# penn-pal-lab/robot_aware_control

Measured on AMD Instinct MI355X. Metric: SVG train frames/sec + CEM candidate-rollouts/sec, 64x64, higher is better.
Workload: dtype fp32 (conv operands as two fp16 parts = 22 significant bits, fp32 accumulate; see fp32_exact)

## Files before the change

### robot_aware_control_amd/csrc/rac_split16.hip

```cpp
#include <math.h>
#include <stdlib.h>

#include <type_traits>

#include "rac_common.h"

namespace rac {

typedef _Float16 f16x8 __attribute__((ext_vector_type(8)));
typedef _Float16 f16x4 __attribute__((ext_vector_type(4)));
typedef unsigned int u32x4 __attribute__((ext_vector_type(4)));
typedef unsigned int u32x2 __attribute__((ext_vector_type(2)));
typedef __amdgpu_buffer_rsrc_t rsrc_t;

constexpr unsigned OOB = 0xFFFFFFF0u;
constexpr int SBN = 128, SBK = 32;

__device__ __forceinline__ const void* uniform_ptr(const void* p) {
  unsigned long long v = reinterpret_cast<unsigned long long>(p);
  unsigned lo = __builtin_amdgcn_readfirstlane((unsigned)v);
  unsigned hi = __builtin_amdgcn_readfirstlane((unsigned)(v >> 32));
  return reinterpret_cast<const void*>(((unsigned long long)hi << 32) | lo);
}
__device__ __forceinline__ rsrc_t make_rsrc(const void* p, unsigned bytes) {
// ... 1535 lines not shown
        __builtin_amdgcn_sched_barrier(0);
        f16x8 fb[NB][2];
#pragma unroll
        for (int j2 = 0; j2 < NT; ++j2)
#pragma unroll
          for (int nb = 0; nb < 2; ++nb)
#pragma unroll
            for (int part = 0; part < 2; ++part)
              fb[j2 * 2 + nb][part] = __builtin_bit_cast(f16x8, bs[tap % 3][(j2 * 2 + part) * 2 + nb]);
        if (!(RAC_EXP_PERSIST & 8) || tap == 0) {
#pragma unroll
          for (int t = HB; t < MB; ++t) read_frag(t, tap, cur * abuf);
        }
        __builtin_amdgcn_sched_barrier(0);
#pragma unroll
        for (int t = 0; t < HB; ++t)
#pragma unroll
          for (int nb = 0; nb < NB; ++nb) acc[t][nb] = mma3(fa[t], fb[nb], acc[t][nb]);
        __builtin_amdgcn_sched_barrier(0);
        if (tap == 8 && more) {
          store_a(cur ^ 1, pow2f(cur_t.ka));
          __syncthreads();
          cur ^= 1;
        }
        if ((tap < 8 || more) && (!(RAC_EXP_PERSIST & 8) || tap == 8)) {
#pragma unroll
          for (int t = 0; t < HB; ++t) read_frag(t, (tap + 1) % 9, cur * abuf);
        }
        __builtin_amdgcn_sched_barrier(0);
#pragma unroll
        for (int t = HB; t < MB; ++t)
#pragma unroll
          for (int nb = 0; nb < NB; ++nb) acc[t][nb] = mma3(fa[t], fb[nb], acc[t][nb]);
      }
    }
    const int img = p.per_image ? cur_t.m0 / p.HW : 0;
    if (RAC_EXP_PERSIST & 2) {
      unsigned mx = 0;
#pragma unroll
      for (int i = 0; i < MB; ++i)
#pragma unroll
        for (int j = 0; j < NB; ++j)
#pragma unroll
          for (int r = 0; r < 4; ++r) mx = max(mx, absbits(acc[i][j][r]));
      if (p.out_amax) amax_commit(mx, p.out_amax + img);
    } else {
      conv16_epilogue(p, acc, cur_t.m0, wm * MB, nmb, n0 + wn * NT * 32, 0, pow2f(-cur_t.ka), pow2f(-kw), pre, nullptr,
                      p.out_amax ? p.out_amax + img : nullptr);
    }
    if (!has_next) break;
    cur ^= 1;
    cur_t = nxt_t;
    bx = next_bx;
  }
}

__global__ __launch_bounds__(256) void absmax_kernel(const float4* x0, long n0v, const float4* x1, long n1v,
                                                     unsigned* amax) {
  __shared__ unsigned sh[4];
  unsigned m = 0;
  const long stride = (long)gridDim.x * blockDim.x;
  for (long i = (long)blockIdx.x * blockDim.x + threadIdx.x; i < n0v + n1v; i += stride) {
    const float4 v = i < n0v ? x0[i] : x1[i - n0v];
    const unsigned a = __builtin_bit_cast(unsigned, v.x) & 0x7FFFFFFFu, b = __builtin_bit_cast(unsigned, v.y) & 0x7FFFFFFFu,
                   c = __builtin_bit_cast(unsigned, v.z) & 0x7FFFFFFFu, d = __builtin_bit_cast(unsigned, v.w) & 0x7FFFFFFFu;
    m = max(m, max(max(a, b), max(c, d)));
  }
#pragma unroll
  for (int o = 32; o > 0; o >>= 1) m = max(m, (unsigned)__shfl_xor((int)m, o));
  if ((threadIdx.x & 63) == 0) sh[threadIdx.x >> 6] = m;
  __syncthreads();
  if (threadIdx.x == 0) {
    m = max(max(sh[0], sh[1]), max(sh[2], sh[3]));
    if (m > __hip_atomic_load(amax, __ATOMIC_RELAXED, __HIP_MEMORY_SCOPE_AGENT)) atomicMax(amax, m);
  }
}

__device__ __forceinline__ void weight_frag16_block(const float* w, const unsigned* w_amax, unsigned short* out, int Cout,
                                                    int Cin, int taps, int transposed, long ps, long block) {
  const int R = transposed ? Cin : Cout, Kc = transposed ? Cout : Cin;
  const int cch = Kc >> 5;
  const long cell = block * 2 + (threadIdx.x >> 7);
  if (cell >= (long)(R >> 5) * cch * taps) return;
  const float s = pow2f(scale_exp(*w_amax));
  const int tap = (int)(cell % taps);
  const int cc = (int)((cell / taps) % cch);
  const int nt = (int)(cell / ((long)taps * cch));
  const int nb = (threadIdx.x >> 6) & 1, lane = threadIdx.x & 63;
  const int r = nt * 32 + nb * 16 + (lane & 15);
  const int k0 = cc * 32 + 8 * (lane >> 4);
  u32x4 lo, hi;
  if (!transposed) {
    const u32x4* src = reinterpret_cast<const u32x4*>(w + ((long)r * taps + tap) * Cin + k0);
    lo = src[0], hi = src[1];
  } else {
    unsigned v[8];
#pragma unroll
    for (int j = 0; j < 8; ++j)
      v[j] = __builtin_bit_cast(unsigned, w[((long)(k0 + j) * taps + (taps - 1 - tap)) * Cin + r]);
    lo = u32x4{v[0], v[1], v[2], v[3]}, hi = u32x4{v[4], v[5], v[6], v[7]};
  }
  u32x4 q[2];
  split8h(lo, hi, s, q);
  const long o = (cell * 2 + nb) * 512 + lane * 8;
  *reinterpret_cast<u32x4*>(out + o) = q[0];
  *reinterpret_cast<u32x4*>(out + ps + o) = q[1];
}

__global__ void weight_frag16_kernel(const float* w, const unsigned* w_amax, unsigned short* out, int Cout, int Cin,
                                     int taps, int transposed, long ps) {
  weight_frag16_block(w, w_amax, out, Cout, Cin, taps, transposed, ps, blockIdx.x);
}

template <typename Job>
__device__ __forceinline__ int job_of_block(const Job* jobs, int n_jobs, long block) {
  int lo = 0, hi = n_jobs - 1;
  while (lo < hi) {
    const int mid = (lo + hi + 1) >> 1;
    if (jobs[mid].block_begin <= block) lo = mid; else hi = mid - 1;
  }
  return lo;
}

__global__ void weight_frag16_multi_kernel(const rac_frag_job* jobs, int n_jobs) {
  const int j = job_of_block(jobs, n_jobs, blockIdx.x);
  const rac_frag_job q = jobs[j];
  weight_frag16_block(q.w, q.w_amax, q.parts, q.Cout, q.Cin, q.ksize * q.ksize, q.transposed, q.part_stride,
                      blockIdx.x - q.block_begin);
}

__global__ __launch_bounds__(256) void absmax_multi_kernel(const rac_absmax_job* jobs, int n_jobs) {
  __shared__ unsigned sh[4];
  const int j = job_of_block(jobs, n_jobs, blockIdx.x);
  const rac_absmax_job q = jobs[j];
  const long nb = (j + 1 < n_jobs ? jobs[j + 1].block_begin : (long)gridDim.x) - q.block_begin;
  const float4* x = reinterpret_cast<const float4*>(q.x);
  const long nv = q.n >> 2;
  unsigned m = 0;
  for (long i = (blockIdx.x - q.block_begin) * 256 + threadIdx.x; i < nv; i += nb * 256) {
    const float4 v = x[i];
    m = max(m, max(max(absbits(v.x), absbits(v.y)), max(absbits(v.z), absbits(v.w))));
  }
#pragma unroll
  for (int o = 32; o > 0; o >>= 1) m = max(m, (unsigned)__shfl_xor((int)m, o));
  if ((threadIdx.x & 63) == 0) sh[threadIdx.x >> 6] = m;
  __syncthreads();
  if (threadIdx.x == 0) {
    m = max(max(sh[0], sh[1]), max(sh[2], sh[3]));
    if (m > __hip_atomic_load(q.amax, __ATOMIC_RELAXED, __HIP_MEMORY_SCOPE_AGENT)) atomicMax(q.amax, m);
  }
}


__global__ __launch_bounds__(256) void adam_frag_multi_kernel(const rac_adam_frag_job* jobs, int n_jobs, long total_blocks,
                                                              float b1, float b2, float eps, float step_size,
                                                              float inv_sqrt_bc2) {
  __shared__ float tile[2][32][33];
  __shared__ unsigned mx_sh[4];
  for (long blk = blockIdx.x; blk < total_blocks; blk += gridDim.x) {
  const int j = job_of_block(jobs, n_jobs, (int)blk);
  const rac_adam_frag_job q = jobs[j];
  const int taps = q.ksize * q.ksize, cch = q.Cin >> 5;
  const int half = threadIdx.x >> 7;
  const long cell = (blk - q.block_begin) * 2 + half;
  const bool active = cell < (long)(q.Cout >> 5) * cch * taps;
  const int tap = (int)(cell % taps);
  const int cc = (int)((cell / taps) % cch);
  const int nt = (int)(cell / ((long)taps * cch));
  const int nb = (threadIdx.x >> 6) & 1, lane = threadIdx.x & 63;
  const int rl = nb * 16 + (lane & 15), kl = 8 * (lane >> 4);
  const float s = pow2f(scale_exp(*q.scale_slot));
  unsigned mx = 0;
  if (active) {
    const long off = ((long)(nt * 32 + rl) * taps + tap) * q.Cin + cc * 32 + kl;
    f32x4 P[2], G[2], M[2], V[2];
#pragma unroll
    for (int h = 0; h < 2; ++h) {
      P[h] = *reinterpret_cast<const f32x4*>(q.p + off + 4 * h);
      G[h] = *reinterpret_cast<const f32x4*>(q.g + off + 4 * h);
      M[h] = *reinterpret_cast<const f32x4*>(q.m + off + 4 * h);
      V[h] = *reinterpret_cast<const f32x4*>(q.v + off + 4 * h);
#pragma unroll
      for (int e = 0; e < 4; ++e) {
        float pp = P[h][e], mm = M[h][e], vv = V[h][e];
        adam_update(pp, G[h][e], mm, vv, b1, b2, eps, step_size, inv_sqrt_bc2);
        M[h][e] = mm, V[h][e] = vv, P[h][e] = pp;
        mx = max(mx, absbits(pp));
        tile[half][rl][kl + 4 * h + e] = pp;
      }
      *reinterpret_cast<f32x4*>(q.p + off + 4 * h) = P[h];
      *reinterpret_cast<f32x4*>(q.m + off + 4 * h) = M[h];
      *reinterpret_cast<f32x4*>(q.v + off + 4 * h) = V[h];
    }
    if (q.parts_fwd) {
      u32x4 parts[2];
      split8h(__builtin_bit_cast(u32x4, P[0]), __builtin_bit_cast(u32x4, P[1]), s, parts);
      const long o = (cell * 2 + nb) * 512 + lane * 8;
      *reinterpret_cast<u32x4*>(q.parts_fwd + o) = parts[0];
      *reinterpret_cast<u32x4*>(q.parts_fwd + q.part_stride + o) = parts[1];
    }
  }
  __syncthreads();
  if (active && q.parts_t) {
    float v[8];
#pragma unroll
    for (int e = 0; e < 8; ++e) v[e] = tile[half][kl + e][rl];
    u32x4 parts[2];
    split8h(u32x4{__builtin_bit_cast(unsigned, v[0]), __builtin_bit_cast(unsigned, v[1]), __builtin_bit_cast(unsigned, v[2]),
                  __builtin_bit_cast(unsigned, v[3])},
            u32x4{__builtin_bit_cast(unsigned, v[4]), __builtin_bit_cast(unsigned, v[5]), __builtin_bit_cast(unsigned, v[6]),
                  __builtin_bit_cast(unsigned, v[7])}, s, parts);
    const long cell_t = ((long)cc * (q.Cout >> 5) + nt) * taps + (taps - 1 - tap);
    const long o = (cell_t * 2 + nb) * 512 + lane * 8;
    *reinterpret_cast<u32x4*>(q.parts_t + o) = parts[0];
    *reinterpret_cast<u32x4*>(q.parts_t + q.part_stride + o) = parts[1];
  }
#pragma unroll
  for (int o = 32; o > 0; o >>= 1) mx = max(mx, (unsigned)__shfl_xor((int)mx, o));
  if (lane == 0) mx_sh[threadIdx.x >> 6] = mx;
  __syncthreads();
  if (threadIdx.x == 0) {
    mx = max(max(mx_sh[0], mx_sh[1]), max(mx_sh[2], mx_sh[3]));
    if (mx > __hip_atomic_load(q.amax_out, __ATOMIC_RELAXED, __HIP_MEMORY_SCOPE_AGENT)) atomicMax(q.amax_out, mx);
  }
  }
}

__global__ void amax_bound_kernel(unsigned* exact, unsigned* bound, const int* idx, int n, float margin) {
  const int j = blockIdx.x * blockDim.x + threadIdx.x;
  if (j >= n) return;
  const int i = idx[j];
  bound[i] = __builtin_bit_cast(unsigned, __builtin_bit_cast(float, exact[i]) + margin);
  exact[i] = 0;
}


struct Wgrad16P {
  int Bimg, H, W, Cin, Cout, C0, T;
  int R, G;
  int nsplit, accumulate;
  int nseg;
  int x1_skip;
  int presplit;
  const float* dy[RAC_WGRAD_MAX_STEPS];
  const float* x0[RAC_WGRAD_MAX_STEPS];
  const float* x1[RAC_WGRAD_MAX_STEPS];
  const unsigned* dy_amax[RAC_WGRAD_MAX_STEPS];
  const unsigned* x0_amax[RAC_WGRAD_MAX_STEPS];
  const unsigned* x1_amax[RAC_WGRAD_MAX_STEPS];
  float* dw;
  float* slabs;
  long slab_stride;
};

typedef __fp16 h16x4 __attribute__((__vector_size__(4 * sizeof(__fp16))));
#define RAC_LDS_PTR(T, base, off) reinterpret_cast<__attribute__((address_space(3))) T*>( \
    (__attribute__((address_space(3))) unsigned char*)(base) + (off))

__device__ __forceinline__ int wg_swz(int r) { return (r & 3) | (((r >> 3) & 1) << 2); }

__device__ __forceinline__ f16x8 tr_frag(const unsigned char* lds, int addr) {
  typedef __fp16 h16x8 __attribute__((__vector_size__(8 * sizeof(__fp16))));
  const h16x4 lo = __builtin_amdgcn_ds_read_tr16_b64_v4f16(RAC_LDS_PTR(h16x4, lds, addr));
  const h16x4 hi = __builtin_amdgcn_ds_read_tr16_b64_v4f16(RAC_LDS_PTR(h16x4, lds, addr + 1024));
  return __builtin_bit_cast(f16x8, (h16x8)__builtin_shufflevector(lo, hi, 0, 1, 2, 3, 4, 5, 6, 7));
}

template <int N>
struct StepPhase {
  static constexpr int v = N;
};
constexpr unsigned OOBV = 0xFFFFFF00u;

__device__ __forceinline__ u32x4 load16s(rsrc_t r, unsigned voff, unsigned soff) {
  return __builtin_bit_cast(u32x4, __builtin_amdgcn_raw_buffer_load_b128(r, (int)voff, (int)soff, 0));
}

template <int KS, int WMW, bool PRE>
__global__ __launch_bounds__(256, 2) void wgrad16_kernel(Wgrad16P p) {
  constexpr int PAD = KS / 2, NR = 2 * PAD + 2;
  constexpr int AHEAD = (KS == 5 && WMW == 2) ? 1 : 2;
  constexpr int DYB = 16384, XSLOT = 8192, X_BASE = 2 * DYB;
  constexpr unsigned EB = PRE ? 2u : 4u;
  static_assert(NR % 2 == 0, "the dy buffer index is a function of the ring phase");
  extern __shared__ __attribute__((aligned(16))) unsigned char lds_raw[];
  const int tid = threadIdx.x;
  const int lane = tid & 63;
  const int wid = __builtin_amdgcn_readfirstlane(tid >> 6);
  constexpr int WN = 4 / WMW, NU = 4 / WN;
  const int wm = wid / WN, wn = wid % WN;
  const int co0 = blockIdx.x * (64 * WMW), ci0 = blockIdx.y * 64;
  const int ky = blockIdx.z % KS, split = blockIdx.z / KS;
  const bool first = ci0 < p.C0;
  const int Cs = first ? p.C0 : p.Cin - p.C0;
  const int cl0 = first ? ci0 : ci0 - p.C0;

  float sd = 1.f, sx = 1.f;
  int kd, kxs;
  {
    unsigned amd = 0, amx = 0;
    for (int t = 0; t < p.T; ++t) {
      amd = max(amd, *p.dy_amax[t]);
      amx = max(amx, *p.x0_amax[t]);
      if (p.x1_amax[t]) amx = max(amx, *p.x1_amax[t]);
    }
    kd = scale_exp(amd), kxs = scale_exp(amx);
    sd = pow2f(kd), sx = pow2f(kxs);
  }

  const int g_skip = first ? 0 : p.x1_skip * p.G;
  const int NG = p.T * p.G;
  const int gpb = (NG - g_skip + p.nsplit - 1) / p.nsplit;
  const int g_begin = g_skip + split * gpb;
  const int g_end = min(NG, g_begin + gpb);
  const int S = max(0, g_end - g_begin) * p.W;

  const int skk = tid >> 3, ssub = tid & 7;
  const int ssw = wg_swz(skk);
  const bool dy_role = WMW == 2 || wid < 2;
  const int dkk = WMW == 2 ? skk : (tid >> 2) & 31, dsub = WMW == 2 ? ssub : tid & 3;
  const int dsw = wg_swz(dkk);
  const int dy_lds = dkk * 256 + ((dsub ^ dsw) * 32);
  const unsigned dflip = (unsigned)(WMW == 2 ? ((dsub ^ dsw) >> 2) & 1 : dkk & 1) * 16u;
  const int x_lds = X_BASE + skk * 256 + (((ssub >> 1) ^ ssw) * 32) + (ssub & 1) * 16;
  const bool dy_ch_ok = co0 + dsub * 16 < p.Cout;
  const bool x_ch_ok = cl0 + ssub * 8 < Cs;

  const unsigned dy_col = (unsigned)p.Cout * EB, dy_row = (unsigned)p.W * dy_col, dy_grp = 32u * dy_row;
  const unsigned dy_part = PRE ? (unsigned)((long)p.R * dy_row) : 0u;
  const unsigned dy_lane = ((unsigned)(dkk * p.W) * (unsigned)p.Cout + (unsigned)(co0 + dsub * 16)) * EB;
  const unsigned d_v0 = dy_ch_ok ? dy_lane + (PRE ? dflip : 2u * dflip) : OOBV;
  const unsigned d_v1 = dy_ch_ok ? dy_lane + (PRE ? (dflip ^ 16u) : (32u ^ (2u * dflip))) : OOBV;
  const unsigned x_col = (unsigned)Cs * EB, x_row = (unsigned)p.W * x_col, x_grp = 32u * x_row;
  const unsigned x_part = PRE ? (unsigned)((long)p.R * x_row) : 0u;
  const unsigned x_lane = ((unsigned)(skk * p.W) * (unsigned)Cs + (unsigned)(cl0 + ssub * 8)) * EB;
  const long x_shift = (long)(ky - PAD) * (long)x_row;
  const bool h32 = __builtin_amdgcn_readfirstlane((32 % p.H) == 0 ? 1 : 0) != 0;
  const bool y_ok0 = (unsigned)(skk % p.H + ky - PAD) < (unsigned)p.H;
  const float* const* xsrc = first ? p.x0 : p.x1;

  int dT = g_begin / p.G, dG = g_begin - dT * p.G, dC = 0;
  int xT = dT, xG = dG, xC = 0;
  rsrc_t d_rs = make_rsrc(p.dy[0], 0u), x_rs = d_rs, d_rs1 = d_rs, x_rs1 = d_rs;
  unsigned d_so = 0, x_so = 0;
  unsigned x_v = (x_ch_ok & (y_ok0 | !h32)) ? x_lane : OOBV;
  u32x4 rdS[AHEAD][4], rxS[AHEAD][2];
  auto issue_dy = [&](u32x4 (&rd)[4]) {
    if (dC == 0) {
      const char* base = reinterpret_cast<const char*>(p.dy[dT]) + (long)dG * dy_grp;
      d_rs = make_rsrc(base, (unsigned)(p.R - dG * 32) * dy_row);
      if constexpr (PRE) d_rs1 = make_rsrc(base + dy_part, (unsigned)(p.R - dG * 32) * dy_row);
      d_so = 0;
    }
    if (dy_role) {
      if constexpr (PRE) {
        rd[0] = load16s(d_rs, d_v0, d_so);
        rd[1] = load16s(d_rs, d_v1, d_so);
        rd[2] = load16s(d_rs1, d_v0, d_so);
        rd[3] = load16s(d_rs1, d_v1, d_so);
      } else {
        rd[0] = load16s(d_rs, d_v0, d_so);
        rd[1] = load16s(d_rs, d_v0 + 16u, d_so);
        rd[2] = load16s(d_rs, d_v1, d_so);
        rd[3] = load16s(d_rs, d_v1 + 16u, d_so);
      }
    }
    d_so += dy_col;
    if (++dC == p.W) {
      dC = 0;
      if (++dG == p.G) dG = 0, ++dT;
    }
  };
  auto issue_x = [&](u32x4 (&rx)[2]) {
    if (xC == 0) {
      const char* base = reinterpret_cast<const char*>(xsrc[xT]) + ((long)xG * x_grp + x_shift);
      x_rs = make_rsrc(base, (unsigned)(p.R - xG * 32) * x_row);
      if constexpr (PRE) x_rs1 = make_rsrc(base + x_part, (unsigned)(p.R - xG * 32) * x_row);
// ... 960 lines not shown
```

### robot_aware_control_amd/ops.py

```python
from __future__ import annotations

import contextlib
import ctypes as C
import functools
import os
import weakref
from typing import Optional, Tuple

import torch

from . import _lib
from ._lib import (AbsmaxJob, AdamFragJob, AdamRange, ConvArgs, FragJob, GradSrc, OptimRange, WgradArgs, call, ptr,
                   stream_ptr)

FWD, DGRAD, WGRAD = 0, 1, 2
ACT_NONE, ACT_LEAKY, ACT_SIGMOID = 0, 1, 2
LOSS_KINDS = {"mse": 0, "l1": 1, "dontcare_mse": 2, "dontcare_l1": 3}
BN_EPS, BN_MOMENTUM = 1e-5, 0.1


def _require_cuda(t: torch.Tensor):
    if not t.is_cuda:
        raise _lib.RacError("robot_aware_control_amd ops run on the GPU only (no CPU fallback); got a CPU tensor")

# ... 243 lines not shown
    M = dy.numel() // dy.shape[-1]
    if _WINDOW is not None and M <= _COLSUM_STEPS_MAX_ROWS:
        _WINDOW.biases.setdefault(id(bias), (bias, []))[1].append(dy)
        return
    call("rac_colsum_acc", ptr(dy), ptr(grad_buffer(bias)), ptr(_colsum_parts(dy.device, M, dy.shape[-1])), M,
         dy.shape[-1], stream_ptr())


def _colsum_parts(device, M: int, Cc: int):
    return torch.empty(int(_lib.load().rac_colsum_blocks(M, Cc)) * Cc, device=device, dtype=torch.float32)


_COLSUM_STEPS_MAX_ROWS = 16384


SPLIT_GEMM = os.environ.get("RAC_SPLIT_GEMM", "1") == "1"
SPLIT_GEMM_TRAIN = SPLIT_GEMM
HEAD_DIRECT = os.environ.get("RAC_HEAD_DIRECT", "1") == "1"
FIRST_MFMA = os.environ.get("RAC_FIRST_MFMA", "1") == "1"
HEAD_DGRAD = os.environ.get("RAC_HEAD_DGRAD", "1") == "1"
HEAD_MFMA = os.environ.get("RAC_HEAD_MFMA", "1") == "1"
SPLIT_MIN_COUT = int(os.environ.get("RAC_SPLIT_MIN_COUT", "64"))
SPLIT_MIN_COUT_TRAIN = int(os.environ.get("RAC_SPLIT_MIN_COUT_TRAIN", "64"))

_AMAX = {"buf": None, "used": 0, "one": None}
_AMAX_SLOTS = 1 << 20


def _amax_take(device, n: int) -> torch.Tensor:
    buf = _AMAX["buf"]
    if buf is None or buf.device != torch.device(device) or _AMAX["used"] + n > _AMAX_SLOTS:
        buf = _AMAX["buf"] = torch.zeros(max(_AMAX_SLOTS, n), device=device, dtype=torch.int32)
        _AMAX["used"] = 0
    k = _AMAX["used"]
    _AMAX["used"] = k + n
    return buf[k:k + n]


def amax_of(x0: torch.Tensor, x1: Optional[torch.Tensor] = None, per_image: bool = False) -> torch.Tensor:
    if per_image:
        assert x1 is None
        slot = _amax_take(x0.device, x0.shape[0])
        call("rac_absmax_rows", ptr(x0), x0.shape[0], x0.numel() // x0.shape[0], ptr(slot), stream_ptr())
        return slot
    slot = _amax_take(x0.device, 1)
    call("rac_absmax", ptr(x0), x0.numel(), ptr(x1), x1.numel() if x1 is not None else 0, ptr(slot), stream_ptr())
    return slot


def amax_slot(device, n: int = 1) -> torch.Tensor:
    return _amax_take(device, n)


def amax_one(device, n: int = 1) -> torch.Tensor:
    one = _AMAX["one"]
    if one is None or one.device != torch.device(device) or one.numel() < n:
        one = _AMAX["one"] = torch.full((max(n, 1024),), 0x3F800000, device=device, dtype=torch.int32)
    view = one[:n]
    view._rac_bound1 = True
    return view


def tag_amax(t: torch.Tensor, slot: torch.Tensor) -> torch.Tensor:
    t._rac_amax = slot
    t._rac_amax_ver = t._version
    return t


def amax_tag(t):
    if t is None or getattr(t, "_rac_amax_ver", None) != t._version:
        return None
    return getattr(t, "_rac_amax", None)


def retag(t, slot):
    if t is not None and slot is not None:
        t._rac_amax = slot
        t._rac_amax_ver = t._version
    return t


def amax_for(t: torch.Tensor, per_image: bool = False) -> torch.Tensor:
    slot = amax_tag(t)
    want = t.shape[0] if per_image else 1
    if slot is not None and getattr(slot, "_rac_bound1", False):
        return amax_one(t.device, want)
    if slot is None or slot.numel() != want:
        slot = amax_of(t, per_image=per_image)
        tag_amax(t, slot)
    return slot


def broadcast_images(t: torch.Tensor, n: int) -> torch.Tensor:
    out = t.expand(n, *t.shape[1:]).contiguous()
    slot = amax_tag(t)
    if slot is not None:
        if getattr(slot, "_rac_bound1", False):
            tag_amax(out, amax_one(t.device, n))
        elif slot.numel() == 1:
            tag_amax(out, slot.expand(n).contiguous())
    return out


_SPLIT_OK = {}


def split_supported(H: int, W: int, k: int, Cin: int, Cout: int, a_split: int = 0) -> bool:
    key = (H, W, k, Cin, Cout, a_split)
    ok = _SPLIT_OK.get(key)
    if ok is None:
        ok = _SPLIT_OK[key] = bool(_lib.load().rac_conv2d_split_supported(H, W, k, Cin, Cout, a_split))
    return ok


class _WeightParts:
    __slots__ = ("ref", "idx", "slot", "device", "parts", "tag", "exact_ok", "__weakref__")


_WP_ENTRIES = {}
_WP_DEV = {}
_WP_NSLOTS = 1024


def _wp_state(device):
    st = _WP_DEV.get(device)
    if st is None:
        st = _WP_DEV[device] = {"slots": torch.zeros(_WP_NSLOTS, device=device, dtype=torch.int32),
                                "exact": torch.zeros(_WP_NSLOTS, device=device, dtype=torch.int32),
                                "free": list(range(_WP_NSLOTS - 1, -1, -1)), "tables": {}, "adam_plan": None,
                                "optim_plan": None}
    return st


def _wp_drop(key, device, idx, _ref):
    ent = _WP_ENTRIES.get(key)
    if ent is not None and ent.idx == idx and ent.device == device:
        del _WP_ENTRIES[key]
        st = _WP_DEV.get(device)
        if st is not None:
            st["free"].append(idx)


def _wp_tag(weight):
    src = getattr(weight, "_rac_sources", None)
    ver = weight._version if src is None else tuple(t._version for t in src)
    return (ver, PARAM_EPOCH, weight.data_ptr())


def _wp_upload(jobs, device):
    raw = bytes(jobs)
    return torch.frombuffer(bytearray(raw), dtype=torch.uint8).to(device)


ADAM_LATE_WGS = int(os.environ.get("RAC_ADAM_LATE_WGS", "512"))
ADAM_WGS = int(os.environ.get("RAC_ADAM_WGS", "0"))


PARAM_GATE = None


def param_wait(t: torch.Tensor = None) -> None:
    gate = PARAM_GATE
    if gate is None:
        return
    if t is None:
        gate.wait_params()
    elif hasattr(gate, "wait_for"):
        gate.wait_for(t)
    elif not gate.ready(t):
        gate.wait_params()


def _wp_tables(st, items, device):
    lib = _lib.load()
    sig = tuple((w.data_ptr(), ent.idx, tuple(sorted((t, q.data_ptr()) for t, q in ent.parts.items())))
                for ent, w in items)
    tables = st["tables"].get(sig)
    if tables is None:
        if len(st["tables"]) > 8:
            st["tables"].clear()
        ajobs = (AbsmaxJob * len(items))()
        nfrag = sum(len(ent.parts) for ent, _ in items)
        fjobs = (FragJob * nfrag)()
        ab = fb = j = 0
        for i, (ent, w) in enumerate(items):
            wm = weight_mem(w.detach())
            co, ci, k, _ = w.shape
            ajobs[i] = AbsmaxJob(x=ptr(wm), n=wm.numel(), amax=ptr(ent.slot), block_begin=ab)
            ab += lib.rac_absmax_blocks(wm.numel())
            for transposed, parts in sorted(ent.parts.items()):
                fjobs[j] = FragJob(w=ptr(wm), w_amax=ptr(ent.slot), parts=ptr(parts), part_stride=wm.numel(), Cout=co,
                                   Cin=ci, ksize=k, transposed=1 if transposed else 0, block_begin=fb)
                fb += lib.rac_weight_frag_blocks(co, ci, k)
                j += 1
        idx = torch.tensor([ent.idx for ent, _ in items], device=device, dtype=torch.long)
        tables = st["tables"][sig] = (_wp_upload(ajobs, device), len(items), ab, _wp_upload(fjobs, device), nfrag, fb, idx)
    return tables


def _wp_refresh(device):
    st = _wp_state(device)
    stale, n_live = [], 0
    gate = PARAM_GATE
    for ent in list(_WP_ENTRIES.values()):
        if ent.device != device:
            continue
        w = ent.ref()
        if w is None:
            continue
        src = getattr(w, "_rac_pad_source", None)
        if gate is not None:
            base = src[0]() if src is not None else w
            if base is not None and not gate.ready(base):
                continue
        if src is not None:
            param = src[0]()
            if param is None:
                continue
            padded_weight(param, src[1])
        n_live += 1
        if ent.tag != _wp_tag(w):
            stale.append((ent, w))
    if not stale:
        return
    sp = stream_ptr()
    if len(stale) <= 2:
        for ent, w in stale:
            ent.slot.zero_()
            wm = weight_mem(w.detach())
            co, ci, k, _ = w.shape
            call("rac_absmax", ptr(wm), wm.numel(), None, 0, ptr(ent.slot), sp)
            for transposed, parts in ent.parts.items():
                call("rac_weight_frag_split", ptr(wm), ptr(ent.slot), ptr(parts), co, ci, k, 1 if transposed else 0,
                     wm.numel(), sp)
            st["exact"][ent.idx:ent.idx + 1].copy_(ent.slot)
            ent.tag, ent.exact_ok = _wp_tag(w), True
        return
    ta, na, ab, tf, nf, fb, idx = _wp_tables(st, stale, device)
    st["slots"].index_fill_(0, idx, 0)
    call("rac_absmax_multi", ptr(ta), na, ab, sp)
    call("rac_weight_frag_split_multi", ptr(tf), nf, fb, sp)
    st["exact"].index_copy_(0, idx, st["slots"].index_select(0, idx))
    for ent, w in stale:
        ent.tag, ent.exact_ok = _wp_tag(w), True


ADAM_FUSED = os.environ.get("RAC_ADAM_FUSED", "1") == "1"
_ADAM_BOUNDS = {}


def adam_step_bound(beta1: float, beta2: float):
    key = (beta1, beta2)
    if key not in _ADAM_BOUNDS:
        r = beta1 * beta1 / beta2
        if not (0.0 <= beta1 < 1.0 and 0.0 < beta2 < 1.0 and r < 1.0):
            _ADAM_BOUNDS[key] = None
        else:
            best, series, b1t, b2t, rk = 0.0, 0.0, 1.0, 1.0, 1.0
            for _ in range(200000):
                series += rk
                rk *= r
                b1t *= beta1
                b2t *= beta2
                best = max(best, (1 - beta1) ** 2 / (1 - b1t) ** 2 * (1 - b2t) / (1 - beta2) * series)
                if rk < 1e-18 and b1t < 1e-18 and b2t < 1e-9:
                    break
            _ADAM_BOUNDS[key] = best ** 0.5
    return _ADAM_BOUNDS[key]


def _wp_covered(flat):
    dev = flat.device
    base, nbytes = flat.data_ptr(), flat.numel() * 4
    covered = []
    for ent in _WP_ENTRIES.values():
        if ent.device != dev:
            continue
        w = ent.ref()
        if w is None or getattr(w, "_rac_pad_source", None) is not None:
            continue
        off = w.data_ptr() - base
        co, ci, k, _ = w.shape
        if not (0 <= off < nbytes and off % 16 == 0 and w.stride() == (k * k * ci, 1, k * ci, ci)):
            continue
        if ent.tag != _wp_tag(w) or not ent.exact_ok:
            return None
        covered.append((off // 4, ent, w))
    covered.sort(key=lambda c: c[0])
    return covered


def fused_adam_step(flat, grad, m, v, lr, beta1, beta2, eps, step, late=None):
    global PARAM_EPOCH
    if not ADAM_FUSED:
        return False
    bound = adam_step_bound(beta1, beta2)
    if bound is None:
        return False
    dev = flat.device
    st = _wp_state(dev)
    base = flat.data_ptr()
    covered = _wp_covered(flat)
    if not covered:
        return False
    late_sets = [] if late is None else (list(late[1]) if isinstance(late[1], (list, tuple)) else [late[1]])

    def late_group(off, w):
# ... 2396 lines not shown
```

Measured before the change: 4133.

## Software-pipeline Adam fragment kernel loads across grid-stride iterations

The Adam fragment kernel's grid-stride loop is restructured so the next block's parameters, gradients and moments are prefetched into registers while the current block is updated. Job lookup is cached and re-seeked only when a block crosses into a new job. The per-block amax reduction and atomic are deferred until the job changes, and the memory access mapping is changed to coalesced row strides. Gradients are loaded and split parts stored with nontemporal hints. The late-launch workgroup count drops from 512 to 256, which gives each workgroup more iterations to pipeline but lowers parallelism and raises register pressure.

Measured after the change: 4166 (median of 4 runs). About the same (+0.8%).

```diff
diff --git a/robot_aware_control_amd/csrc/rac_split16.hip b/robot_aware_control_amd/csrc/rac_split16.hip
--- a/robot_aware_control_amd/csrc/rac_split16.hip
+++ b/robot_aware_control_amd/csrc/rac_split16.hip
@@ -1711,77 +1711,147 @@
 }
 
 
-__global__ __launch_bounds__(256) void adam_frag_multi_kernel(const rac_adam_frag_job* jobs, int n_jobs, long total_blocks,
-                                                              float b1, float b2, float eps, float step_size,
-                                                              float inv_sqrt_bc2) {
+__device__ __forceinline__ void adam_barrier() {
+  __builtin_amdgcn_fence(__ATOMIC_RELEASE, "workgroup");
+  __builtin_amdgcn_s_barrier();
+  __builtin_amdgcn_fence(__ATOMIC_ACQUIRE, "workgroup");
+}
+__device__ __forceinline__ unsigned adam_lane_xor(unsigned v, int o) {
+  return (unsigned)__builtin_amdgcn_ds_bpermute((int)(((threadIdx.x & 63) ^ o) << 2), (int)v);
+}
+template <typename T, typename U>
+__device__ __forceinline__ __attribute__((address_space(1))) T* gmem(U* p) {
+  return (__attribute__((address_space(1))) T*)p;
+}
+
+struct adam_walk {
+  rac_adam_frag_job q;
+  long end;
+  float s;
+  int j;
+};
+struct adam_cell {
+  long cell, off, step;
+  int tap, cc, nt;
+  bool active;
+};
+struct adam_regs {
+  f32x4 P[2], G[2], M[2], V[2];
+};
+
+__device__ __forceinline__ void adam_walk_seek(adam_walk& w, const rac_adam_frag_job* __restrict__ jobs, int n_jobs,
+                                               long total_blocks, long blk) {
+  w.j = job_of_block(jobs, n_jobs, blk);
+  w.q = jobs[w.j];
+  w.end = w.j + 1 < n_jobs ? jobs[w.j + 1].block_begin : total_blocks;
+  w.s = pow2f(scale_exp(*gmem<const unsigned>(w.q.scale_slot)));
+}
+
+__device__ __forceinline__ adam_cell adam_cell_of(const rac_adam_frag_job& q, long blk, int half, int lr, int lc) {
+  adam_cell c;
+  const unsigned taps = q.ksize * q.ksize, cch = q.Cin >> 5;
+  const unsigned cell = (unsigned)(blk - q.block_begin) * 2u + half;
+  c.active = cell < (unsigned long)(q.Cout >> 5) * cch * taps;
+  c.tap = (int)(cell % taps), c.cc = (int)((cell / taps) % cch), c.nt = (int)(cell / (taps * cch));
+  c.cell = cell;
+  c.off = ((long)(c.nt * 32 + lr) * taps + c.tap) * q.Cin + c.cc * 32 + lc;
+  c.step = 16L * taps * q.Cin;
+  return c;
+}
+
+__device__ __forceinline__ void adam_fetch(adam_regs& d, const rac_adam_frag_job& q, const adam_cell& c) {
+  if (!c.active) return;
+#pragma unroll
+  for (int h = 0; h < 2; ++h) {
+    const long o = c.off + h * c.step;
+    d.P[h] = *gmem<const f32x4>(q.p + o);
+    d.G[h] = __builtin_nontemporal_load(gmem<const f32x4>(q.g + o));
+    d.M[h] = *gmem<const f32x4>(q.m + o);
+    d.V[h] = *gmem<const f32x4>(q.v + o);
+  }
+}
+
+__device__ __forceinline__ void adam_parts_out(const float (*tile)[33], bool t, int rl, int kl, float s, unsigned short* out,
+                                               long part_stride, long o) {
+  unsigned v[8];
+#pragma unroll
+  for (int e = 0; e < 8; ++e) v[e] = __builtin_bit_cast(unsigned, t ? tile[kl + e][rl] : tile[rl][kl + e]);
+  u32x4 parts[2];
+  split8h(u32x4{v[0], v[1], v[2], v[3]}, u32x4{v[4], v[5], v[6], v[7]}, s, parts);
+  __builtin_nontemporal_store(parts[0], gmem<u32x4>(out + o));
+  __builtin_nontemporal_store(parts[1], gmem<u32x4>(out + part_stride + o));
+}
+
+__global__ __launch_bounds__(256) void adam_frag_multi_kernel(const rac_adam_frag_job* __restrict__ jobs, int n_jobs,
+                                                              long total_blocks, float b1, float b2, float eps,
+                                                              float step_size, float inv_sqrt_bc2) {
   __shared__ float tile[2][32][33];
   __shared__ unsigned mx_sh[4];
-  for (long blk = blockIdx.x; blk < total_blocks; blk += gridDim.x) {
-  const int j = job_of_block(jobs, n_jobs, (int)blk);
-  const rac_adam_frag_job q = jobs[j];
-  const int taps = q.ksize * q.ksize, cch = q.Cin >> 5;
-  const int half = threadIdx.x >> 7;
-  const long cell = (blk - q.block_begin) * 2 + half;
-  const bool active = cell < (long)(q.Cout >> 5) * cch * taps;
-  const int tap = (int)(cell % taps);
-  const int cc = (int)((cell / taps) % cch);
-  const int nt = (int)(cell / ((long)taps * cch));
-  const int nb = (threadIdx.x >> 6) & 1, lane = threadIdx.x & 63;
+  const int half = threadIdx.x >> 7, nb = (threadIdx.x >> 6) & 1, lane = threadIdx.x & 63;
   const int rl = nb * 16 + (lane & 15), kl = 8 * (lane >> 4);
-  const float s = pow2f(scale_exp(*q.scale_slot));
+  const int lr = (threadIdx.x & 127) >> 3, lc = 4 * (threadIdx.x & 7);
+  long blk = blockIdx.x;
+  if (blk >= total_blocks) return;
+  adam_walk wn;
+  adam_walk_seek(wn, jobs, n_jobs, total_blocks, blk);
+  adam_cell cn = adam_cell_of(wn.q, blk, half, lr, lc);
+  adam_regs dn{};
+  adam_fetch(dn, wn.q, cn);
   unsigned mx = 0;
-  if (active) {
-    const long off = ((long)(nt * 32 + rl) * taps + tap) * q.Cin + cc * 32 + kl;
-    f32x4 P[2], G[2], M[2], V[2];
-#pragma unroll
-    for (int h = 0; h < 2; ++h) {
-      P[h] = *reinterpret_cast<const f32x4*>(q.p + off + 4 * h);
-      G[h] = *reinterpret_cast<const f32x4*>(q.g + off + 4 * h);
-      M[h] = *reinterpret_cast<const f32x4*>(q.m + off + 4 * h);
-      V[h] = *reinterpret_cast<const f32x4*>(q.v + off + 4 * h);
-#pragma unroll
-      for (int e = 0; e < 4; ++e) {
-        float pp = P[h][e], mm = M[h][e], vv = V[h][e];
-        adam_update(pp, G[h][e], mm, vv, b1, b2, eps, step_size, inv_sqrt_bc2);
-        M[h][e] = mm, V[h][e] = vv, P[h][e] = pp;
-        mx = max(mx, absbits(pp));
-        tile[half][rl][kl + 4 * h + e] = pp;
-      }
-      *reinterpret_cast<f32x4*>(q.p + off + 4 * h) = P[h];
-      *reinterpret_cast<f32x4*>(q.m + off + 4 * h) = M[h];
-      *reinterpret_cast<f32x4*>(q.v + off + 4 * h) = V[h];
-    }
-    if (q.parts_fwd) {
-      u32x4 parts[2];
-      split8h(__builtin_bit_cast(u32x4, P[0]), __builtin_bit_cast(u32x4, P[1]), s, parts);
-      const long o = (cell * 2 + nb) * 512 + lane * 8;
-      *reinterpret_cast<u32x4*>(q.parts_fwd + o) = parts[0];
-      *reinterpret_cast<u32x4*>(q.parts_fwd + q.part_stride + o) = parts[1];
-    }
-  }
-  __syncthreads();
-  if (active && q.parts_t) {
-    float v[8];
-#pragma unroll
-    for (int e = 0; e < 8; ++e) v[e] = tile[half][kl + e][rl];
-    u32x4 parts[2];
-    split8h(u32x4{__builtin_bit_cast(unsigned, v[0]), __builtin_bit_cast(unsigned, v[1]), __builtin_bit_cast(unsigned, v[2]),
-                  __builtin_bit_cast(unsigned, v[3])},
-            u32x4{__builtin_bit_cast(unsigned, v[4]), __builtin_bit_cast(unsigned, v[5]), __builtin_bit_cast(unsigned, v[6]),
-                  __builtin_bit_cast(unsigned, v[7])}, s, parts);
-    const long cell_t = ((long)cc * (q.Cout >> 5) + nt) * taps + (taps - 1 - tap);
-    const long o = (cell_t * 2 + nb) * 512 + lane * 8;
-    *reinterpret_cast<u32x4*>(q.parts_t + o) = parts[0];
-    *reinterpret_cast<u32x4*>(q.parts_t + q.part_stride + o) = parts[1];
-  }
-#pragma unroll
-  for (int o = 32; o > 0; o >>= 1) mx = max(mx, (unsigned)__shfl_xor((int)mx, o));
-  if (lane == 0) mx_sh[threadIdx.x >> 6] = mx;
-  __syncthreads();
-  if (threadIdx.x == 0) {
-    mx = max(max(mx_sh[0], mx_sh[1]), max(mx_sh[2], mx_sh[3]));
-    if (mx > __hip_atomic_load(q.amax_out, __ATOMIC_RELAXED, __HIP_MEMORY_SCOPE_AGENT)) atomicMax(q.amax_out, mx);
-  }
+  for (;;) {
+    const adam_walk w = wn;
+    const adam_cell c = cn;
+    adam_regs d = dn;
+    const rac_adam_frag_job& q = w.q;
+    const long nblk = blk + gridDim.x;
+    const bool more = nblk < total_blocks;
+    if (more) {
+      if (nblk >= wn.end) adam_walk_seek(wn, jobs, n_jobs, total_blocks, nblk);
+      cn = adam_cell_of(wn.q, nblk, half, lr, lc);
+      adam_fetch(dn, wn.q, cn);
+    }
+    const int taps = q.ksize * q.ksize;
+    if (c.active) {
+#pragma unroll
+      for (int h = 0; h < 2; ++h) {
+#pragma unroll
+        for (int e = 0; e < 4; ++e) {
+          float pp = d.P[h][e], mm = d.M[h][e], vv = d.V[h][e];
+          adam_update(pp, d.G[h][e], mm, vv, b1, b2, eps, step_size, inv_sqrt_bc2);
+          d.M[h][e] = mm, d.V[h][e] = vv, d.P[h][e] = pp;
+          mx = max(mx, absbits(pp));
+          tile[half][lr + 16 * h][lc + e] = pp;
+        }
+        const long o = c.off + h * c.step;
+        *gmem<f32x4>(q.p + o) = d.P[h];
+        *gmem<f32x4>(q.m + o) = d.M[h];
+        *gmem<f32x4>(q.v + o) = d.V[h];
+      }
+    }
+    adam_barrier();
+    if (c.active && q.parts_fwd)
+      adam_parts_out(tile[half], false, rl, kl, w.s, q.parts_fwd, q.part_stride, (c.cell * 2 + nb) * 512 + lane * 8);
+    if (c.active && q.parts_t) {
+      const long cell_t = ((long)c.cc * (q.Cout >> 5) + c.nt) * taps + (taps - 1 - c.tap);
+      adam_parts_out(tile[half], true, rl, kl, w.s, q.parts_t, q.part_stride, (cell_t * 2 + nb) * 512 + lane * 8);
+    }
+    const bool flush = !more || wn.j != w.j;
+    if (flush) {
+#pragma unroll
+      for (int o = 32; o > 0; o >>= 1) mx = max(mx, adam_lane_xor(mx, o));
+      if (lane == 0) mx_sh[threadIdx.x >> 6] = mx;
+    }
+    adam_barrier();
+    if (flush) {
+      if (threadIdx.x == 0) {
+        mx = max(max(mx_sh[0], mx_sh[1]), max(mx_sh[2], mx_sh[3]));
+        if (mx > __hip_atomic_load(q.amax_out, __ATOMIC_RELAXED, __HIP_MEMORY_SCOPE_AGENT))
+          __hip_atomic_fetch_max(q.amax_out, mx, __ATOMIC_RELAXED, __HIP_MEMORY_SCOPE_AGENT);
+      }
+      mx = 0;
+    }
+    if (!more) break;
+    blk = nblk;
   }
 }
 
diff --git a/robot_aware_control_amd/ops.py b/robot_aware_control_amd/ops.py
--- a/robot_aware_control_amd/ops.py
+++ b/robot_aware_control_amd/ops.py
@@ -419,7 +419,7 @@
     return torch.frombuffer(bytearray(raw), dtype=torch.uint8).to(device)
 
 
-ADAM_LATE_WGS = int(os.environ.get("RAC_ADAM_LATE_WGS", "512"))
+ADAM_LATE_WGS = int(os.environ.get("RAC_ADAM_LATE_WGS", "256"))
 ADAM_WGS = int(os.environ.get("RAC_ADAM_WGS", "0"))
 
 
```
